# rustformers/llm

Hardware: NVIDIA B200
Metric: LLaMA-7B Q4_0 tokens/sec (decode@1, n_past=512) (higher is better)
Workload: dtype u8/s8 block dots -> f32 (Q4_0 weights x Q8_0 activations)

## Files before the change

llm_b200/csrc/decode_ops.cu:

```cuda
#include <cooperative_groups.h>
#include <stdlib.h>

#include <array>
#include <map>
#include <vector>

#include "decode.h"
#include "stream_core.cuh"
#include "tp.cuh"

namespace b200 {

using namespace stream;

__constant__ TpCtx c_tp;

namespace {

__device__ __forceinline__ unsigned long long gtime() { unsigned long long t; asm volatile("mov.u64 %0, %%globaltimer;" : "=l"(t)); return t; }
__device__ __forceinline__ void prof_begin(unsigned long long *p) { if (p && threadIdx.x == 0) { const unsigned long long t = gtime(); atomicMin(p, t); atomicMax(p + 3 * B200_PROF_SLOTS, t); } }
__device__ __forceinline__ void prof_ready(unsigned long long *p) { if (p && threadIdx.x == 0) { const unsigned long long t = gtime(); atomicMin(p + 2 * B200_PROF_SLOTS, t); atomicMax(p + 4 * B200_PROF_SLOTS, t); } }
__device__ __forceinline__ void prof_end(unsigned long long *p) { if (p && threadIdx.x == 0) atomicMax(p + B200_PROF_SLOTS, gtime()); }

__device__ __forceinline__ void pdl_trigger() { asm volatile("griddepcontrol.launch_dependents;" ::: "memory"); }
__device__ __forceinline__ void pdl_wait() { asm volatile("griddepcontrol.wait;" ::: "memory"); }

int pdl_mask() {
    static int mask = -1;
    if (mask < 0) { const char *e = getenv("B200_PDL"); mask = e ? atoi(e) : 3; }
    return mask;
}

template <int CLASS = 2, typename... KArgs, typename... Args>
void launch_k(void (*kern)(KArgs...), dim3 grid, dim3 block, size_t smem, cudaStream_t st, Args &&...args) {
    cudaLaunchConfig_t cfg{};
    cfg.gridDim = grid; cfg.blockDim = block; cfg.dynamicSmemBytes = smem; cfg.stream = st;
    cudaLaunchAttribute at[1];
    at[0].id = cudaLaunchAttributeProgrammaticStreamSerialization;
    at[0].val.programmaticStreamSerializationAllowed = 1;
    cfg.attrs = at; cfg.numAttrs = (pdl_mask() & CLASS) ? 1 : 0;
    B200_CHECK(cudaLaunchKernelEx(&cfg, kern, KArgs(args)...));
}

__device__ __forceinline__ float lutf(const uint16_t *t, float x) { return f16_bits_to_f32(__ldg(t + f32_to_f16_bits(x))); }
__device__ __forceinline__ float f16dot_tree(float s) {
    s = __fadd_rn(s, __shfl_down_sync(0xffffffffu, s, 16));
    s = __fadd_rn(s, __shfl_down_sync(0xffffffffu, s, 8));
    s = __fadd_rn(s, __shfl_down_sync(0xffffffffu, s, 4));
    s = __fadd_rn(s, __shfl_down_sync(0xffffffffu, s, 1));
    s = __fadd_rn(s, __shfl_down_sync(0xffffffffu, s, 2));
    return s;
}

template <bool TP>
__device__ __forceinline__ void norm_pack_body(const float *__restrict__ x, const float *__restrict__ gain, int4 *__restrict__ pack,
                                               int e, float eps, int q81, int off, int scale16, unsigned long long *prof, const TpSync &S) {
    const TpCtx &T = c_tp;
    __shared__ double shd[8];
    const int tid = threadIdx.x, lane = tid & 31, warp = tid >> 5;
    pdl_trigger();
    if (!(TP && (T.relax & 1))) pdl_wait();
    constexpr bool tp = TP;
    const unsigned tag = tp ? tp_tag(T, S.in_v) : 0u;

    prof_begin(prof);
    const int mine = blockIdx.x * 256 + tid, nv = e / 4;
    const bool active = mine < nv;
    const float4 gv = active ? __ldg((const float4 *)gain + mine) : make_float4(0.f, 0.f, 0.f, 0.f);
    float4 xv = make_float4(0.f, 0.f, 0.f, 0.f);
    double s = 0.0;
    constexpr int U = 4;
    if (tp && (T.relax & 1)) {
        if (warp == 0) tp_wait_sample(T, S.in_buf, (int64_t)e, tag, lane);
        __syncthreads();
    }
    for (int i0 = tid; i0 < nv; i0 += 256 * U) {
        float4 v[U];
        if (!tp) {
#pragma unroll
            for (int k = 0; k < U; k++) { const int i = i0 + 256 * k; v[k] = i < nv ? __ldcg((const float4 *)x + i) : make_float4(0.f, 0.f, 0.f, 0.f); }
        } else {
            uint4 ra[U], rb[U];
#pragma unroll
// ... 269 lines not shown
#pragma unroll
    for (int cc = 0; cc < 8; cc++) acc[cc] = 0.f;
    for (int k0 = 0; k0 < np; k0 += KC) {
        __syncthreads();
#pragma unroll
        for (int u = 0; u < KC / 32; u++) ((int4 *)vt)[tid + u * 128] = pre[u];
        __syncthreads();
        if (k0 + KC < np) fetch(k0 + KC);
        const int kend = np - k0 < KC ? np - k0 : KC;
#pragma unroll
        for (int cc = 0; cc < 8; cc++) {
            const __half *vrow = vt + (warp * 8 + cc) * KC;
            for (int k = lane; k < kend; k += 32) acc[cc] = __fmaf_rn(__half2float(vrow[k]), __half2float(p16[k0 + k]), acc[cc]);
        }
    }
    __syncthreads();
#pragma unroll
    for (int cc = 0; cc < 8; cc++) {
        const float a = f16dot_tree(acc[cc]);
        if (lane == 0) {
            const __half *vrow = vleft + (warp * 8 + cc) * 32;
            double sumf = (double)a;
            for (int k = np; k < n_kv; k++) sumf += (double)__fmul_rn(__half2float(vrow[k - np]), __half2float(p16[k]));
            stash[warp * 8 + cc] = (float)sumf;
        }
    }
    __syncthreads();
    if (warp == 0) pack_quad(((const float4 *)stash)[lane & 7], xpack_out + (int64_t)((h * hd + c0) / QK) * 4, lane, lane < 8, q81, off, scale16);
    prof_end(prof);
}

__device__ __forceinline__ float quad_tree(float (&acc)[8]) {
#pragma unroll
    for (int e = 0; e < 8; e++) acc[e] = __fadd_rn(acc[e], __shfl_xor_sync(0xffffffffu, acc[e], 2));
#pragma unroll
    for (int e = 0; e < 8; e++) acc[e] = __fadd_rn(acc[e], __shfl_xor_sync(0xffffffffu, acc[e], 1));
    const float r0 = __fadd_rn(acc[0], acc[4]), r1 = __fadd_rn(acc[1], acc[5]), r2 = __fadd_rn(acc[2], acc[6]), r3 = __fadd_rn(acc[3], acc[7]);
    return __fadd_rn(__fadd_rn(r0, r1), __fadd_rn(r2, r3));
}
__device__ __forceinline__ void fma8(float (&acc)[8], const int4 &a, const int4 &b) {
    const __half2 *ah = (const __half2 *)&a, *bh = (const __half2 *)&b;
#pragma unroll
    for (int e = 0; e < 4; e++) {
        const float2 af = __half22float2(ah[e]), bf = __half22float2(bh[e]);
        acc[2 * e] = __fmaf_rn(af.x, bf.x, acc[2 * e]); acc[2 * e + 1] = __fmaf_rn(af.y, bf.y, acc[2 * e + 1]);
    }
}

constexpr int ATH = 256;
template <bool TP>
__global__ void __launch_bounds__(ATH) attn_fused_kernel(const float *__restrict__ q, const __half *__restrict__ Kl, const __half *__restrict__ Vl,
                                                         int4 *__restrict__ xpack_out, const int *__restrict__ n_past, const uint16_t *__restrict__ lut_exp,
                                                         float kq_scale, int hd, int n_head, int n_head_kv, int gqa, int n_ctx, int nlay, int q81, int off, int scale16,
                                                         unsigned long long *prof, const TpSync S, int head0) {
    const TpCtx &T = c_tp;
    namespace cg = cooperative_groups;
    cg::cluster_group cluster = cg::this_cluster();
    extern __shared__ __align__(16) uint8_t sm[];
    __shared__ double shd[ATH / 32];
    __shared__ float shf[ATH / 32], stash[32];
    prof_begin(prof);
    const int per_head = hd / 32, h = blockIdx.x / per_head, part = blockIdx.x - h * per_head, c0 = part * 32;
    const int hk = h / (n_head / n_head_kv);
    const int tid = threadIdx.x, lane = tid & 31, warp = tid >> 5, u = tid & 3;
    const int vstride = nlay + 32;
    float *sc = (float *)sm;
    __half *p16 = (__half *)(sm + (size_t)nlay * 4);
    __half *q16 = p16 + nlay;
    __half *vs = (__half *)(sm + (((size_t)nlay * 6 + (size_t)hd * 2 + 127) & ~(size_t)127));
    pdl_trigger();
    pdl_wait();
    float qv = 0.f;
    if (tid < hd) qv = __ldcg(q + h * hd + tid);
    const int n_kv = __ldcg(n_past) + 1;
    const int np = n_kv & ~31;

    {
        const int cpr = (n_kv + 7) / 8;
        for (int i = tid; i < 32 * cpr; i += ATH) {
            const int rr = i / cpr, cc = i - rr * cpr;
            cp16(smem_u32(vs + rr * vstride + cc * 8), Vl + (int64_t)(hk * hd + c0 + rr) * n_ctx + cc * 8);
        }
    }
    if (tid < hd) q16[tid] = __float2half_rn(qv);
    __syncthreads();
    asm volatile("barrier.cluster.arrive.relaxed.aligned;\n\tbarrier.cluster.wait.aligned;" ::: "memory");

    {
        const int per = (n_kv + per_head - 1) / per_head, j0 = part * per, j1 = n_kv < j0 + per ? n_kv : j0 + per;
        const int nvec = hd / 32;
        constexpr int PU = 4;
        for (int jb = j0; jb < j1; jb += PU * (ATH / 4)) {
            int4 kv[PU][4];
#pragma unroll
            for (int pu = 0; pu < PU; pu++) {
                const int j = jb + pu * (ATH / 4) + (tid >> 2);
                const __half *krow = Kl + (int64_t)(j < j1 ? j : j0) * gqa + hk * hd + 8 * u;
#pragma unroll
                for (int i = 0; i < 4; i++) if (i < nvec) kv[pu][i] = j < j1 ? __ldcg((const int4 *)(krow + 32 * i)) : make_int4(0, 0, 0, 0);
            }
#pragma unroll
            for (int pu = 0; pu < PU; pu++) {
                const int j = jb + pu * (ATH / 4) + (tid >> 2);
                float acc[8];
#pragma unroll
                for (int e = 0; e < 8; e++) acc[e] = 0.f;
#pragma unroll
                for (int i = 0; i < 4; i++) if (i < nvec) fma8(acc, kv[pu][i], *(const int4 *)(q16 + 32 * i + 8 * u));
                const float s = quad_tree(acc);
                if (j < j1 && u < per_head) cluster.map_shared_rank(sc, u)[j] = __fmul_rn(s, kq_scale);
            }
        }
    }
    cluster.sync();

    float mx = -INFINITY;
    for (int j = tid; j < n_kv; j += ATH) mx = fmaxf(mx, sc[j]);
    mx = warp_max(mx);
    if (lane == 0) shf[warp] = mx;
    __syncthreads();
    mx = shf[0];
#pragma unroll
    for (int i = 1; i < ATH / 32; i++) mx = fmaxf(mx, shf[i]);
    double s = 0.0;
    constexpr int SB = 4;
    for (int jb = 0; jb < n_kv; jb += SB * ATH) {
        uint16_t ev16[SB];
#pragma unroll
        for (int k = 0; k < SB; k++) { const int j = jb + tid + k * ATH; ev16[k] = j < n_kv ? __ldg(lut_exp + f32_to_f16_bits(__fsub_rn(sc[j], mx))) : (uint16_t)0; }
#pragma unroll
        for (int k = 0; k < SB; k++) { const int j = jb + tid + k * ATH; if (j < n_kv) { const float ev = f16_bits_to_f32(ev16[k]); sc[j] = ev; s += (double)ev; } }
    }
    s = warp_sum(s);
    if (lane == 0) shd[warp] = s;
    __syncthreads();
    const float inv = (float)(1.0 / (((shd[0] + shd[1]) + (shd[2] + shd[3])) + ((shd[4] + shd[5]) + (shd[6] + shd[7]))));
    for (int j = tid; j < n_kv; j += ATH) p16[j] = __float2half_rn(__fmul_rn(sc[j], inv));
    asm volatile("cp.async.wait_all;" ::: "memory");
    __syncthreads();

    if (tid < 128) {
        const int col = tid >> 2;
        const __half *vrow = vs + col * vstride;
        float acc[8];
#pragma unroll
        for (int e = 0; e < 8; e++) acc[e] = 0.f;
#pragma unroll 4
        for (int k = 0; k < np; k += 32) fma8(acc, *(const int4 *)(vrow + k + 8 * u), *(const int4 *)(p16 + k + 8 * u));
        const float a = quad_tree(acc);
        if (u == 0) {
            double sumf = (double)a;
            for (int k = np; k < n_kv; k++) sumf += (double)__fmul_rn(__half2float(vrow[k]), __half2float(p16[k]));
            stash[col] = (float)sumf;
        }
    }
    __syncthreads();
    if (warp == 0) {
        int4 rec;
        const int64_t blk = (int64_t)(((head0 + h) * hd + c0) / QK);
        if (pack_quad_rec(((const float4 *)stash)[lane & 7], lane, lane < 8, q81, off, scale16, rec)) {
            if (TP) tp_put_rec(T, TPB_XD, blk * 4 + (lane & 7), rec, tp_tag(T, S.out_v)); else xpack_out[blk * 4 + (lane & 7)] = rec;
        }
    }
    prof_end(prof);
}

template <int TYPE, int EPI, bool TP = false>
void launch_mmv(const QWeight &w, MmvArgs A, cudaStream_t st) {
    constexpr int ROWS = SR, CB = SCB;
    using T = St<TYPE>;
    static int smem_set = 0, sms = 0, depth_cap = -1;
    static std::map<int, std::array<int, SST_MAX + 1>> occ_by_nb;
    if (!sms) { int dev; B200_CHECK(cudaGetDevice(&dev)); B200_CHECK(cudaDeviceGetAttribute(&sms, cudaDevAttrMultiProcessorCount, dev)); }
    if (depth_cap < 0) { const char *e = getenv("B200_RING_DEPTH"); depth_cap = e ? atoi(e) : SST_MAX; if (depth_cap < 2) depth_cap = 2; if (depth_cap > SST_MAX) depth_cap = SST_MAX; }
    auto smem_of = [&](int nst) { return 256 + T::ring_bytes(nst) + (int)w.nb * 64 + 256; };
    if (smem_of(SST_MAX) > smem_set) {
        const int want = smem_of(SST_MAX) < 227 * 1024 ? smem_of(SST_MAX) : 227 * 1024;
        B200_CHECK(cudaFuncSetAttribute(mmv_fused_kernel<TYPE, EPI, TP>, cudaFuncAttributeMaxDynamicSharedMemorySize, want));
        smem_set = smem_of(SST_MAX);
    }
    auto it = occ_by_nb.find((int)w.nb);
    if (it == occ_by_nb.end()) {
        std::array<int, SST_MAX + 1> o{};
        for (int nst = 2; nst <= SST_MAX; nst++)
            if (smem_of(nst) <= 227 * 1024) B200_CHECK(cudaOccupancyMaxActiveBlocksPerMultiprocessor(&o[nst], mmv_fused_kernel<TYPE, EPI, TP>, STHREADS, smem_of(nst)));
        it = occ_by_nb.emplace((int)w.nb, o).first;
    }
    const std::array<int, SST_MAX + 1> &occ = it->second;
    constexpr int G = EPI == EPI_SILU ? 2 : 1;
    const int64_t groups = ((w.N + ROWS - 1) / ROWS + G - 1) / G;
// ... 38 lines not shown
    if (threadIdx.x == 0) *T.epoch = *(volatile unsigned *)T.epoch + 1;
}

template <int TYPE, bool TP>
void decode_ops_t(const DecodeParams &P, const std::vector<DecodeLayer> &layers, int n_kv_bucket, int4 *xpack_a, cudaStream_t st, int *launches) {
    const int q81 = has_min(TYPE) ? 1 : 0, off = TYPE == T_Q5_0 ? 16 : 0, s16 = TYPE == T_Q4_0 ? 1 : 0;
    const int e = P.e, f = P.f;
    const TpCtx &T = P.tp;
    constexpr bool tp = TP;
    B200_ASSERT(tp == (T.world > 1));
    const int e_loc = tp ? P.e_loc : e;
    auto ts = [&](int in_buf, unsigned in_v, int add_buf, unsigned add_v, int out_buf, unsigned out_v) {
        TpSync S;
        if (tp) { S.in_buf = in_buf; S.in_v = in_v; S.add_buf = add_buf; S.add_v = add_v; S.out_buf = out_buf; S.out_v = out_v; }
        return S;
    };
    int n = 0;
    auto pr = [&]() -> unsigned long long * { return P.prof && n < B200_PROF_SLOTS ? P.prof + n : nullptr; };
    auto launch_norm = [&](const float *x, const float *gain, const TpSync &S) {
        const dim3 grid((e / QK + 31) / 32), block(256);
        if constexpr (TP) launch_k(norm_pack_tp_kernel, grid, block, 0, st, x, gain, xpack_a, e, P.eps, q81, off, s16, pr(), S);
        else { (void)S; launch_k(norm_pack_kernel, grid, block, 0, st, x, gain, xpack_a, e, P.eps, q81, off, s16, pr()); }
        n++;
    };
    get_rows_q(P.wte, P.token, P.x, 1, st); n++;
    if (tp) { launch_k(tp_spread_kernel, dim3((e + 255) / 256), dim3(256), 0, st, (const float *)P.x, e); n++; }
    static const bool fused_env = !(getenv("B200_ATTN_FUSED") && getenv("B200_ATTN_FUSED")[0] == '0');
    const int nlay = (n_kv_bucket + 63) / 64 * 64;
    const size_t fa_smem = (((size_t)nlay * 6 + (size_t)P.hd * 2 + 127) & ~(size_t)127) + (size_t)32 * (nlay + 32) * 2;
    const bool fused_attn = (fused_env || tp) && P.hd % 32 == 0 && P.hd <= 128 && P.n_ctx % 8 == 0 && fa_smem <= 227 * 1024;
    B200_ASSERT(fused_attn || !tp);
    if (fused_attn) attn_fused_reserve(fa_smem);
    const size_t sv_smem = (size_t)P.n_ctx * 6 + 32 * KC * 2 + 32 * 32 * 2;
    static size_t sv_set = 48 * 1024;
    if (sv_smem > sv_set) { B200_CHECK(cudaFuncSetAttribute(attn_sv_kernel, cudaFuncAttributeMaxDynamicSharedMemorySize, (int)sv_smem)); sv_set = sv_smem; }
    for (int il = 0; il < P.n_layer; il++) {
        const DecodeLayer &L = layers[il];
        const unsigned v = (unsigned)il + 1;
        launch_norm(P.x, L.attn_norm, ts(TPB_X, (unsigned)il, -1, 0, -1, 0));
        MmvArgs A{}; A.xpack = xpack_a; A.q = P.q; A.K = L.K; A.V = L.V; A.rope_cs = P.rope_cs; A.rope_half = P.rope_half; A.hd = P.hd; A.e = e_loc; A.gqa = P.gqa;
        A.n_ctx = P.n_ctx; A.n_past = P.n_past;
        A.prof = pr(); launch_mmv<TYPE, EPI_QKV, TP>(L.wqkv, A, st); n++;
        if (fused_attn) {
            cudaLaunchConfig_t cfg{};
            cfg.gridDim = dim3(P.n_head * (P.hd / 32)); cfg.blockDim = dim3(ATH); cfg.dynamicSmemBytes = fa_smem; cfg.stream = st;
            cudaLaunchAttribute at[2];
            at[0].id = cudaLaunchAttributeClusterDimension;
            at[0].val.clusterDim.x = P.hd / 32; at[0].val.clusterDim.y = 1; at[0].val.clusterDim.z = 1;
            at[1].id = cudaLaunchAttributeProgrammaticStreamSerialization;
            at[1].val.programmaticStreamSerializationAllowed = 1;
            cfg.attrs = at; cfg.numAttrs = (pdl_mask() & 2) ? 2 : 1;
            B200_CHECK(cudaLaunchKernelEx(&cfg, attn_fused_kernel<TP>, (const float *)P.q, (const __half *)L.K, (const __half *)L.V, P.xpack_d, (const int *)P.n_past,
                                          (const uint16_t *)P.lut_exp, P.kq_scale, P.hd, P.n_head, P.n_head_kv, P.gqa, P.n_ctx, nlay, q81, off, s16, pr(),
                                          ts(-1, 0, -1, 0, TPB_XD, v), tp ? P.head0 : 0));
            n++;
        } else {
            launch_k(P.hd == 128 ? attn_kq_kernel<128> : attn_kq_kernel<64>, dim3((n_kv_bucket + 63) / 64, P.n_head), dim3(128), 0, st,
                     P.q, L.K, P.kq, P.n_past, P.gqa, P.n_head, P.n_head_kv, P.n_ctx, pr());
            n++;
            launch_k(attn_sv_kernel, dim3(P.n_head * (P.hd / 32)), dim3(128), sv_smem, st, P.kq, L.V, P.xpack_d, P.n_past, P.lut_exp, P.kq_scale, P.hd, P.n_head,
                     P.n_head_kv, P.n_ctx, q81, off, s16, pr()); n++;
        }
        MmvArgs Bo{}; Bo.xpack = P.xpack_d; Bo.dst = P.ff; Bo.addend = P.x;
        Bo.ts = ts(TPB_XD, v, TPB_X, (unsigned)il, TPB_FF, v); Bo.row0 = tp ? P.row0_e : 0;
        Bo.prof = pr(); launch_mmv<TYPE, EPI_RES, TP>(L.wo, Bo, st); n++;
        launch_norm(P.ff, L.ffn_norm, ts(TPB_FF, v, -1, 0, -1, 0));
        MmvArgs C{}; C.xpack = xpack_a; C.xpack_out = P.xpack_f; C.lut_silu = P.lut_silu; C.q81 = q81; C.off = off; C.scale16 = s16;
        C.ts = ts(-1, 0, -1, 0, TPB_XF, v); C.row0 = tp ? P.row0_w13 : 0;
        C.prof = pr(); launch_mmv<TYPE, EPI_SILU, TP>(L.w13, C, st); n++;
        MmvArgs D{}; D.xpack = P.xpack_f; D.dst = P.x; D.addend = P.ff;
        D.ts = ts(TPB_XF, v, TPB_FF, v, TPB_X, v); D.row0 = tp ? P.row0_e : 0;
        D.prof = pr(); launch_mmv<TYPE, EPI_RES, TP>(L.w2, D, st); n++;
    }
    launch_norm(P.x, P.norm, ts(TPB_X, (unsigned)P.n_layer, -1, 0, -1, 0));
    MmvArgs Z{}; Z.xpack = xpack_a; Z.dst = P.logits; Z.addend = nullptr; Z.n_past_inc = P.n_past;
    Z.ts = ts(-1, 0, -1, 0, TPB_LOGITS, 0); Z.row0 = tp ? P.row0_v : 0;
    Z.prof = pr(); launch_mmv<TYPE, EPI_LOGITS, TP>(P.output, Z, st); n++;
    if (tp) {
        launch_k(tp_collect_kernel, dim3((P.n_vocab_full + 255) / 256), dim3(256), 0, st, P.logits, P.n_vocab_full); n++;
        launch_k(tp_bump_kernel, dim3(1), dim3(32), 0, st); n++;
    }
    B200_CHECK(cudaGetLastError());
    (void)f;
    if (launches) *launches = n;
}

__global__ void __launch_bounds__(256) ln_pack_kernel(const float *__restrict__ x, const float *__restrict__ gain, const float *__restrict__ bias, int4 *__restrict__ pack,
                                                      int e, int q81, int off, int scale16) {
    __shared__ double shd[8];
    const int tid = threadIdx.x, lane = tid & 31, warp = tid >> 5;
    pdl_trigger();
    pdl_wait();
    constexpr int MAXV = 8;
    const int nv = e / 4, mine = blockIdx.x * 256 + tid;
    float4 v[MAXV];
#pragma unroll
    for (int k = 0; k < MAXV; k++) { const int i = tid + k * 256; v[k] = i < nv ? __ldcg((const float4 *)x + i) : make_float4(0.f, 0.f, 0.f, 0.f); }
    const bool active = mine < nv;
    const float4 gv = active ? __ldg((const float4 *)gain + mine) : make_float4(0.f, 0.f, 0.f, 0.f);
    const float4 bv = active ? __ldg((const float4 *)bias + mine) : make_float4(0.f, 0.f, 0.f, 0.f);
    auto total = [&](double s) {
        s = warp_sum(s);
        __syncthreads();
        if (lane == 0) shd[warp] = s;
        __syncthreads();
        return ((shd[0] + shd[1]) + (shd[2] + shd[3])) + ((shd[4] + shd[5]) + (shd[6] + shd[7]));
    };
// ... 32 lines not shown
    if (n_rot > 0) {
        const int hb = n_rot / 2, ib = c / n_rot, r = c - ib * n_rot;
        if (ib < hd / n_rot) {
            const bool lo = r < hb;
            const int partner = lo ? c + hb : c - hb;
            const float2 cs = __ldg(rope_cs + (int64_t)p * rope_half + ib * hb + (lo ? r : r - hb));
            const float qp = __ldcg(base + partner), kp = __ldcg(base + k_off + partner);
            qo = lo ? __fmaf_rn(qo, cs.x, -__fmul_rn(qp, cs.y)) : __fmaf_rn(qp, cs.y, __fmul_rn(qo, cs.x));
            ko = lo ? __fmaf_rn(ko, cs.x, -__fmul_rn(kp, cs.y)) : __fmaf_rn(kp, cs.y, __fmul_rn(ko, cs.x));
        }
    }
    q[i] = qo;
    Kl[(int64_t)p * e + i] = __float2half_rn(ko);
    Vl[(int64_t)i * n_ctx + p] = __float2half_rn(__ldcg(base + v_off + c));
}

__global__ void __launch_bounds__(256) gpt2_add_pos_kernel(float *__restrict__ x, const float *__restrict__ wpe, const int *__restrict__ n_past, int e) {
    pdl_wait();
    const int i = blockIdx.x * 256 + threadIdx.x;
    if (i < e) x[i] = __fadd_rn(x[i], __ldg(wpe + (int64_t)__ldcg(n_past) * e + i));
}

template <int TYPE>
void neox_ops_t(const NeoxParams &P, const std::vector<NeoxLayer> &layers, int n_kv_bucket, cudaStream_t st, int *launches) {
    const int q81 = has_min(TYPE) ? 1 : 0, off = TYPE == T_Q5_0 ? 16 : 0, s16 = TYPE == T_Q4_0 ? 1 : 0;
    const int e = P.e;
    int n = 0;
    get_rows_q(P.wte, P.token, P.x, 1, st); n++;
    if (P.wpe) { launch_k(gpt2_add_pos_kernel, dim3((e + 255) / 256), dim3(256), 0, st, P.x, P.wpe, (const int *)P.n_past, e); n++; }
    const int nlay = (n_kv_bucket + 63) / 64 * 64;
    const size_t fa_smem = (((size_t)nlay * 6 + (size_t)P.hd * 2 + 127) & ~(size_t)127) + (size_t)32 * (nlay + 32) * 2;
    B200_ASSERT(P.hd % 32 == 0 && P.hd <= 128 && P.n_ctx % 8 == 0 && fa_smem <= 227 * 1024 && e <= 8192);
    attn_fused_reserve(fa_smem);
    const dim3 ln_grid((e / 4 + 255) / 256);
    const TpSync S{};
    for (int il = 0; il < P.n_layer; il++) {
        const NeoxLayer &L = layers[il];
        launch_k(ln_pack_kernel, ln_grid, dim3(256), 0, st, (const float *)P.x, L.ln1_g, L.ln1_b, P.xpack_a, e, q81, off, s16); n++;
        MmvArgs A{}; A.xpack = P.xpack_a; A.dst = P.qkv; A.bias = L.bqkv;
        launch_mmv<TYPE, EPI_BIAS>(L.wqkv, A, st); n++;
        launch_k(neox_rope_store_kernel, dim3((e + 255) / 256), dim3(256), 0, st, (const float *)P.qkv, P.q, L.K, L.V, (const int *)P.n_past, P.rope_cs, P.rope_half,
                 P.gpt2 ? 0 : P.n_rot, P.hd, e, P.n_ctx, P.gpt2 ? P.hd : 3 * P.hd, P.gpt2 ? e : P.hd, P.gpt2 ? 2 * e : 2 * P.hd); n++;
        {
            cudaLaunchConfig_t cfg{};
            cfg.gridDim = dim3(P.n_head * (P.hd / 32)); cfg.blockDim = dim3(ATH); cfg.dynamicSmemBytes = fa_smem; cfg.stream = st;
            cudaLaunchAttribute at[2];
            at[0].id = cudaLaunchAttributeClusterDimension;
            at[0].val.clusterDim.x = P.hd / 32; at[0].val.clusterDim.y = 1; at[0].val.clusterDim.z = 1;
            at[1].id = cudaLaunchAttributeProgrammaticStreamSerialization;
            at[1].val.programmaticStreamSerializationAllowed = 1;
            cfg.attrs = at; cfg.numAttrs = (pdl_mask() & 2) ? 2 : 1;
            B200_CHECK(cudaLaunchKernelEx(&cfg, attn_fused_kernel<false>, (const float *)P.q, (const __half *)L.K, (const __half *)L.V, P.xpack_d, (const int *)P.n_past,
                                          (const uint16_t *)P.lut_exp, P.kq_scale, P.hd, P.n_head, P.n_head, e, P.n_ctx, nlay, q81, off, s16,
                                          (unsigned long long *)nullptr, S, 0));
            n++;
        }
        MmvArgs Bo{}; Bo.xpack = P.xpack_d; Bo.dst = P.attn_out; Bo.bias = L.bdense; Bo.add1 = P.parallel_residual ? nullptr : P.x;
        launch_mmv<TYPE, EPI_BIAS>(L.wdense, Bo, st); n++;
        launch_k(ln_pack_kernel, ln_grid, dim3(256), 0, st, (const float *)(P.parallel_residual ? P.x : P.attn_out), L.ln2_g, L.ln2_b, P.xpack_a, e, q81, off, s16); n++;
        MmvArgs C{}; C.xpack = P.xpack_a; C.xpack_out = P.xpack_f; C.bias = L.bfc; C.lut_gelu = P.lut_gelu; C.q81 = q81; C.off = off; C.scale16 = s16;
        launch_mmv<TYPE, EPI_GELU>(L.wfc, C, st); n++;
        MmvArgs D{}; D.xpack = P.xpack_f; D.dst = P.x; D.bias = L.bproj; D.add1 = P.attn_out; D.add2 = P.parallel_residual ? P.x : nullptr;
        launch_mmv<TYPE, EPI_BIAS>(L.wproj, D, st); n++;
    }
    launch_k(ln_pack_kernel, ln_grid, dim3(256), 0, st, (const float *)P.x, P.lnf_g, P.lnf_b, P.xpack_a, e, q81, off, s16); n++;
    MmvArgs Z{}; Z.xpack = P.xpack_a; Z.dst = P.logits; Z.n_past_inc = P.n_past;
    launch_mmv<TYPE, EPI_BIAS>(P.lm_head, Z, st); n++;
    B200_CHECK(cudaGetLastError());
    if (launches) *launches = n;
}

}

void neox_decode_enqueue(const NeoxParams &P, const std::vector<NeoxLayer> &layers, int wtype, int n_kv_bucket, cudaStream_t st, int *launches) {
    switch (wtype) {
        case T_Q4_0: neox_ops_t<T_Q4_0>(P, layers, n_kv_bucket, st, launches); break;
        case T_Q4_1: neox_ops_t<T_Q4_1>(P, layers, n_kv_bucket, st, launches); break;
        case T_Q5_0: neox_ops_t<T_Q5_0>(P, layers, n_kv_bucket, st, launches); break;
        case T_Q5_1: neox_ops_t<T_Q5_1>(P, layers, n_kv_bucket, st, launches); break;
        case T_Q8_0: neox_ops_t<T_Q8_0>(P, layers, n_kv_bucket, st, launches); break;
        default: B200_ASSERT(!"neox_decode_enqueue: unsupported weight type");
    }
}

void decode_set_tp(const TpCtx &T, cudaStream_t st) {
    B200_CHECK(cudaStreamSynchronize(st));
    B200_CHECK(cudaMemcpyToSymbol(c_tp, &T, sizeof(TpCtx)));
    B200_CHECK(cudaDeviceSynchronize());
}

void decode_ops_enqueue(const DecodeParams &P, const std::vector<DecodeLayer> &layers, int wtype, int n_kv_bucket, int4 *xpack_a, cudaStream_t st, int *launches) {
    const bool tp = P.tp.world > 1;
    switch (wtype) {
        case T_Q4_0: if (tp) decode_ops_t<T_Q4_0, true>(P, layers, n_kv_bucket, xpack_a, st, launches); else decode_ops_t<T_Q4_0, false>(P, layers, n_kv_bucket, xpack_a, st, launches); break;
        case T_Q4_1: if (tp) decode_ops_t<T_Q4_1, true>(P, layers, n_kv_bucket, xpack_a, st, launches); else decode_ops_t<T_Q4_1, false>(P, layers, n_kv_bucket, xpack_a, st, launches); break;
        case T_Q5_0: if (tp) decode_ops_t<T_Q5_0, true>(P, layers, n_kv_bucket, xpack_a, st, launches); else decode_ops_t<T_Q5_0, false>(P, layers, n_kv_bucket, xpack_a, st, launches); break;
        case T_Q5_1: if (tp) decode_ops_t<T_Q5_1, true>(P, layers, n_kv_bucket, xpack_a, st, launches); else decode_ops_t<T_Q5_1, false>(P, layers, n_kv_bucket, xpack_a, st, launches); break;
        case T_Q8_0: if (tp) decode_ops_t<T_Q8_0, true>(P, layers, n_kv_bucket, xpack_a, st, launches); else decode_ops_t<T_Q8_0, false>(P, layers, n_kv_bucket, xpack_a, st, launches); break;
        default: B200_ASSERT(!"decode_ops_enqueue: unsupported weight type");
    }
}

}
```

llm_b200/csrc/session.cu:

```cuda
#include <string.h>

#include <string>
#include <vector>

#include "../../include/llm_b200.h"
#include "decode.h"
#include "kernels.cuh"
#include "runtime.h"

namespace b200 {
void synth_qweight(const QWeight &w, uint64_t seed, cudaStream_t st);
void synth_gain(float *g, int64_t n, uint64_t seed, cudaStream_t st);
}
using namespace b200;

namespace {

QWeight row_view(const QWeight &w, int64_t row0, int64_t nrows) {
    QWeight v = w;
    v.N = nrows;
    v.qs = w.qs + (size_t)row0 * w.nb * qs_bytes(w.type);
    if (w.qh) v.qh = w.qh + (size_t)row0 * w.nb;
    v.dm = (const uint8_t *)w.dm + (size_t)row0 * w.nb * (has_min(w.type) ? 4 : 2);
    v.base = nullptr;
// ... 437 lines not shown
        B200_CHECK(cudaStreamSynchronize(R.stream));
    } else {
        if (nbytes != (size_t)s.n * 4) return B200_ERR_TENSOR_SHAPE;
        B200_CHECK(cudaStreamSynchronize(R.stream));
        B200_CHECK(cudaMemcpy(host_out, s.f, nbytes, cudaMemcpyDeviceToHost));
    }
    return B200_OK;
}

int b200_model_synthesize(b200_model *m, uint64_t seed) {
    if (!m || m->tp_world > 1) return B200_ERR_BAD_ARG;
    cudaStream_t st = rt().stream;
    uint64_t id = 0;
    auto q = [&](const QWeight &w) { synth_qweight(w, seed + 0x1000003ull * (++id), st); };
    auto g = [&](float *p, int64_t n) { synth_gain(p, n, seed + 0x1000003ull * (++id), st); };
    q(m->wte); g(m->norm, m->hp.n_embd); q(m->output);
    for (auto &L : m->layers) { g(L.attention_norm, m->hp.n_embd); g(L.ffn_norm, m->hp.n_embd); q(L.wqkv); q(L.wo); q(L.w13); q(L.w2); }
    B200_CHECK(cudaStreamSynchronize(st));
    m->loaded.assign(m->n_slots(), 1);
    m->n_loaded = m->n_slots();
    return B200_OK;
}

int b200_model_is_loaded(b200_model *m) { return m && m->n_loaded == m->n_slots(); }

void b200_model_free(b200_model *m) {
    if (!m) return;
    B200_CHECK(cudaStreamSynchronize(rt().stream));
    if (m->slab) B200_CHECK(cudaFree(m->slab));
    delete m;
}

static b200_session *start_session_tp(b200_session *s) {
    b200_model *m = s->m;
    const b200_llama_hparams &hp = m->hp;
    const int G = m->tp_world, r = m->tp_rank;
    const size_t e = hp.n_embd, f = hp.n_ff, n_ctx = hp.context_size, gqa = m->gqa_loc, V = hp.n_vocab;
    s->cfg.n_batch = s->cfg.n_batch < 1 ? 1 : s->cfg.n_batch;
    const size_t kv_elems = (size_t)hp.n_layer * n_ctx * gqa;
    B200_CHECK(cudaMalloc(&s->memory_k, kv_elems * 2));
    B200_CHECK(cudaMalloc(&s->memory_v, kv_elems * 2));
    B200_CHECK(cudaMemset(s->memory_k, 0, kv_elems * 2));
    B200_CHECK(cudaMemset(s->memory_v, 0, kv_elems * 2));
    B200_CHECK(cudaMalloc(&s->d_tokens, (size_t)s->cfg.n_batch * 4));
    B200_CHECK(cudaMallocHost(&s->h_tokens, (size_t)s->cfg.n_batch * 4));
    B200_CHECK(cudaMallocHost(&s->h_logits, (size_t)s->cfg.n_batch * V * 4));
    B200_CHECK(cudaMallocHost(&s->h_topk, 2048 * 4));
    B200_CHECK(cudaMalloc(&s->topk, 2048 * 4));
    B200_CHECK(cudaEventCreateWithFlags(&s->tokens_uploaded, cudaEventDisableTiming));
    B200_CHECK(cudaMalloc(&s->qbuf, (size_t)m->e_loc * 4));
    B200_CHECK(cudaMalloc(&s->xpack_a, (e / QK) * 64));
    B200_CHECK(cudaMalloc(&s->d_n_past, sizeof(int)));
    B200_CHECK(cudaMallocHost(&s->h_n_past, sizeof(int)));
    B200_CHECK(cudaMalloc(&s->d_prof, B200_PROF_SLOTS * 8 * sizeof(unsigned long long)));
    B200_CHECK(cudaMemset(s->d_prof, 0, B200_PROF_SLOTS * 8 * sizeof(unsigned long long)));
    TpCtx &T = s->dp.tp;
    T = TpCtx();
    T.world = G; T.rank = r; T.vmul = (unsigned)hp.n_layer + 1;
    { const char *e = getenv("B200_TP_RELAX"); T.relax = e ? atoi(e) : 0; }
    size_t off = 0;
    auto piece = [&](size_t units) { const size_t o = off; off += (units * 8 + 255) & ~(size_t)255; return (uint32_t)o; };
    T.off[TPB_X] = piece(e); T.off[TPB_FF] = piece(e); T.off[TPB_XD] = piece((e / QK) * 16); T.off[TPB_XF] = piece((f / QK) * 16); T.off[TPB_LOGITS] = piece(V);
    s->tp_slab_bytes = off;
    B200_CHECK(cudaMalloc(&s->tp_slab, off));
    B200_CHECK(cudaMemset(s->tp_slab, 0, off));
    B200_CHECK(cudaMalloc(&s->tp_state, 2 * sizeof(unsigned)));
    B200_CHECK(cudaMemset(s->tp_state, 0, 2 * sizeof(unsigned)));
    T.epoch = s->tp_state;
    for (int p = 0; p < TP_MAX; p++) T.peer[p] = nullptr;
    T.peer[r] = s->tp_slab;
    B200_CHECK(cudaMalloc(&s->x, e * 4));
    B200_CHECK(cudaMalloc(&s->logits, V * 4));
    s->ff = nullptr; s->xpack_d = nullptr; s->xpack_f = nullptr;
    const RopeTable &rt_ = rope_table(hp.n_rot, 0, hp.rope_freq_base, hp.rope_freq_scale, m->hd, (int)n_ctx);
    {
        std::vector<DecodeLayer> hl(hp.n_layer);
        for (int il = 0; il < hp.n_layer; il++) {
            const Layer &L = m->layers[il];
            hl[il] = DecodeLayer{L.wqkv, L.wo, L.w13, L.w2, L.attention_norm, L.ffn_norm,
                                 s->memory_k + (size_t)il * n_ctx * gqa, s->memory_v + (size_t)il * n_ctx * gqa};
        }
        s->h_layers = hl;
    }
    DecodeParams &P = s->dp;
    P.layers = nullptr; P.n_layer = hp.n_layer; P.wte = m->wte; P.output = m->output; P.norm = m->norm;
    P.e = (int)e; P.f = m->f_loc; P.hd = m->hd; P.gqa = m->gqa_loc; P.n_head = hp.n_head / G; P.n_head_kv = hp.n_head_kv / G; P.n_ctx = (int)n_ctx; P.n_vocab = m->v_loc;
    P.kq_scale = 1.0f / sqrtf((float)hp.n_embd / (float)hp.n_head); P.eps = 5e-6f;
    P.rope_cs = rt_.cs; P.rope_half = rt_.half;
    P.lut_silu = luts().silu; P.lut_exp = luts().exp;
    P.token = s->d_tokens; P.n_past = s->d_n_past;
    P.x = s->x; P.q = s->qbuf; P.kq = nullptr; P.attn = nullptr; P.ff = s->ff; P.h13 = nullptr; P.logits = s->logits;
    P.xpack_d = s->xpack_d; P.xpack_f = s->xpack_f; P.bar = nullptr; P.scratch_bytes = 0;
    P.e_loc = m->e_loc; P.head0 = r * (hp.n_head / G); P.n_vocab_full = hp.n_vocab;
    P.row0_e = (int64_t)r * m->e_loc; P.row0_w13 = (int64_t)r * 2 * m->f_loc; P.row0_v = (int64_t)r * m->v_loc;
    P.prof = nullptr;
    QWeight probe; probe.nb = (int64_t)e / QK;
    QWeight probe2; probe2.nb = (int64_t)f / QK;
    s->mega_ok = hp.n_rot == m->hd && (m->hd == 64 || m->hd == 128) && mmv_exact_stream_supported(probe) && mmv_exact_stream_supported(probe2) &&
                 m->gqa_loc % 32 == 0 && m->e_loc % 32 == 0 && hp.context_size % 8 == 0;
    B200_CHECK(cudaDeviceSynchronize());
    if (!s->mega_ok) { fprintf(stderr, "llm_b200: tensor-parallel session: geometry not supported by the fused decode schedule\n"); b200_session_free(s); return nullptr; }
    return s;
}

b200_session *b200_model_start_session(b200_model *m, const b200_session_config *cfg) {
    if (!m || !cfg || cfg->n_batch < 1) return nullptr;
    if (m->n_loaded != m->n_slots()) { fprintf(stderr, "llm_b200: start_session: %d of %d tensors loaded\n", m->n_loaded, m->n_slots()); return nullptr; }
    b200_session *s = new b200_session();
// ... 7 lines not shown
    B200_CHECK(cudaMemset(s->memory_k, 0, kv_elems * 2));
    B200_CHECK(cudaMemset(s->memory_v, 0, kv_elems * 2));
    const size_t kmax = e > f ? e : f;
    B200_CHECK(cudaMalloc(&s->d_tokens, B * 4));
    B200_CHECK(cudaMalloc(&s->x, B * e * 4));
    B200_CHECK(cudaMalloc(&s->cur, B * e * 4));
    B200_CHECK(cudaMalloc(&s->ff, B * e * 4));
    B200_CHECK(cudaMalloc(&s->qkv, B * (e + 2 * gqa) * 4));
    B200_CHECK(cudaMalloc(&s->kq, (size_t)hp.n_head * B * n_ctx * 4));
    B200_CHECK(cudaMalloc(&s->h13, B * 2 * f * 4));
    B200_CHECK(cudaMalloc(&s->hmul, B * f * 4));
    B200_CHECK(cudaMalloc(&s->logits, B * (size_t)hp.n_vocab * 4));
    B200_CHECK(cudaMalloc(&s->xq, B * kmax));
    B200_CHECK(cudaMalloc(&s->topk, 2048 * 4));
    B200_CHECK(cudaMalloc(&s->xds, B * (kmax / QK) * sizeof(float2)));
    B200_CHECK(cudaMalloc(&s->xpack, (kmax / QK) * 64));
    B200_CHECK(cudaMalloc(&s->xh, xh_bytes(kmax, B)));
    B200_CHECK(cudaMallocHost(&s->h_tokens, B * 4));
    B200_CHECK(cudaMallocHost(&s->h_logits, B * (size_t)hp.n_vocab * 4));
    B200_CHECK(cudaMallocHost(&s->h_topk, 2048 * 4));
    B200_CHECK(cudaEventCreateWithFlags(&s->tokens_uploaded, cudaEventDisableTiming));
    const RopeTable &rt_ = rope_table(hp.n_rot, 0, hp.rope_freq_base, hp.rope_freq_scale, m->hd, (int)n_ctx);
    B200_CHECK(cudaMalloc(&s->qbuf, e * 4));
    B200_CHECK(cudaMalloc(&s->attn, e * 4));
    B200_CHECK(cudaMalloc(&s->d_bar, 2 * sizeof(unsigned int)));
    B200_CHECK(cudaMemset(s->d_bar, 0, 2 * sizeof(unsigned int)));
    B200_CHECK(cudaMalloc(&s->d_n_past, sizeof(int)));
    B200_CHECK(cudaMallocHost(&s->h_n_past, sizeof(int)));
    {
        std::vector<DecodeLayer> hl(hp.n_layer);
        for (int il = 0; il < hp.n_layer; il++) {
            const Layer &L = m->layers[il];
            hl[il] = DecodeLayer{L.wqkv, L.wo, L.w13, L.w2, L.attention_norm, L.ffn_norm,
                                 s->memory_k + (size_t)il * n_ctx * gqa, s->memory_v + (size_t)il * n_ctx * gqa};
        }
        s->h_layers = hl;
        B200_CHECK(cudaMalloc(&s->d_layers, hl.size() * sizeof(DecodeLayer)));
        B200_CHECK(cudaMemcpy(s->d_layers, hl.data(), hl.size() * sizeof(DecodeLayer), cudaMemcpyHostToDevice));
    }
    DecodeParams &P = s->dp;
    P.layers = s->d_layers; P.n_layer = hp.n_layer; P.wte = m->wte; P.output = m->output; P.norm = m->norm;
    P.e = (int)e; P.f = (int)f; P.hd = m->hd; P.gqa = m->gqa; P.n_head = hp.n_head; P.n_head_kv = hp.n_head_kv; P.n_ctx = (int)n_ctx; P.n_vocab = hp.n_vocab;
    P.kq_scale = 1.0f / sqrtf((float)hp.n_embd / (float)hp.n_head); P.eps = 5e-6f;
    P.rope_cs = rt_.cs; P.rope_half = rt_.half;
    P.lut_silu = luts().silu; P.lut_exp = luts().exp;
    P.token = s->d_tokens; P.n_past = s->d_n_past;
    P.x = s->x; P.q = s->qbuf; P.kq = s->kq; P.attn = s->attn; P.ff = s->ff; P.h13 = s->h13; P.logits = s->logits;
    P.bar = s->d_bar;
    B200_CHECK(cudaMalloc(&s->xpack_d, (e / QK) * 64));
    B200_CHECK(cudaMalloc(&s->xpack_f, (f / QK) * 64));
    P.xpack_d = s->xpack_d; P.xpack_f = s->xpack_f;
    B200_CHECK(cudaMalloc(&s->xpack_a, (e / QK) * 64));
    P.scratch_bytes = decode_scratch_bytes((int)e, (int)f, m->hd, (int)n_ctx);
    B200_CHECK(cudaMalloc(&s->d_prof, B200_PROF_SLOTS * 8 * sizeof(unsigned long long)));
    B200_CHECK(cudaMemset(s->d_prof, 0, B200_PROF_SLOTS * 8 * sizeof(unsigned long long)));
    P.prof = getenv("B200_DECODE_PROF") ? s->d_prof : nullptr;
    s->mega_ok = hp.n_rot == m->hd && (m->hd == 64 || m->hd == 128) && decode_supported(P, hp.wtype);
    B200_CHECK(cudaDeviceSynchronize());
    return s;
}

int32_t b200_session_n_past(const b200_session *s) { return s ? s->n_past : -1; }
int b200_session_set_n_past(b200_session *s, int32_t n_past) {
    if (!s || n_past < 0 || n_past > s->n_past) return B200_ERR_BAD_ARG;
    s->n_past = n_past;
    return B200_OK;
}
int32_t b200_session_last_launches(const b200_session *s) { return s ? s->last_launches : 0; }

int b200_session_evaluate_device(b200_session *s, const int32_t *d_tokens, int32_t n) {
    if (!s || n < 1 || n > s->cfg.n_batch) return B200_ERR_BAD_ARG;
    if (s->n_past + n > s->m->hp.context_size) return B200_ERR_CONTEXT_FULL;
    if (d_tokens && d_tokens != s->d_tokens)
        B200_CHECK(cudaMemcpyAsync(s->d_tokens, d_tokens, (size_t)n * 4, cudaMemcpyDeviceToDevice, rt().stream));
    forward(s, n);
    return B200_OK;
}
const float *b200_session_device_logits(b200_session *s) { return s ? s->logits : nullptr; }

int b200_session_evaluate(b200_session *s, const int32_t *tokens, int32_t n, float *logits_out, int32_t all_logits) {
    if (!s || !tokens || n < 1 || n > s->cfg.n_batch) return B200_ERR_BAD_ARG;
    if (s->n_past + n > s->m->hp.context_size) return B200_ERR_CONTEXT_FULL;
    if (s->m->tp_world > 1 && n > 1) {
        const size_t V = s->m->hp.n_vocab;
        for (int i = 0; i < n; i++) {
            float *out = !logits_out ? nullptr : all_logits ? logits_out + (size_t)i * V : (i == n - 1 ? logits_out : nullptr);
            const int rc = b200_session_evaluate(s, tokens + i, 1, out, 0);
            if (rc != B200_OK) return rc;
        }
        return B200_OK;
    }
    for (int i = 0; i < n; i++) if (tokens[i] < 0 || tokens[i] >= s->m->hp.n_vocab) return B200_ERR_BAD_ARG;
    cudaStream_t st = rt().stream;
    B200_CHECK(cudaEventSynchronize(s->tokens_uploaded));
    memcpy(s->h_tokens, tokens, (size_t)n * 4);
    B200_CHECK(cudaMemcpyAsync(s->d_tokens, s->h_tokens, (size_t)n * 4, cudaMemcpyHostToDevice, st));
    B200_CHECK(cudaEventRecord(s->tokens_uploaded, st));
    forward(s, n, all_logits != 0);
    const size_t V = s->m->hp.n_vocab;
    if (logits_out) {
        const size_t rows = all_logits ? n : 1;
        const float *src = all_logits ? s->logits : s->logits + (size_t)(n - 1) * V;
        B200_CHECK(cudaMemcpyAsync(s->h_logits, src, rows * V * 4, cudaMemcpyDeviceToHost, st));
        B200_CHECK(cudaStreamSynchronize(st));
        memcpy(logits_out, s->h_logits, rows * V * 4);
    }
    return B200_OK;
}
// ... 8 lines not shown
    B200_CHECK(cudaMemcpyAsync(s->h_topk, d_ids, (size_t)k * 4, cudaMemcpyDeviceToHost, st));
    B200_CHECK(cudaMemcpyAsync(s->h_topk + 1024, d_vals, (size_t)k * 4, cudaMemcpyDeviceToHost, st));
    B200_CHECK(cudaStreamSynchronize(st));
    memcpy(ids_out, s->h_topk, (size_t)k * 4);
    memcpy(logits_out, s->h_topk + 1024, (size_t)k * 4);
    return B200_OK;
}

int b200_session_feed_prompt(b200_session *s, const int32_t *tokens, int32_t n, float *last_logits_out) {
    if (!s || !tokens || n < 0) return B200_ERR_BAD_ARG;
    if (s->n_past + n > s->m->hp.context_size) return B200_ERR_CONTEXT_FULL;
    for (int i = 0; i < n; i += s->cfg.n_batch) {
        const int c = (n - i) < s->cfg.n_batch ? (n - i) : s->cfg.n_batch;
        const bool last = i + c >= n;
        const int rc = b200_session_evaluate(s, tokens + i, c, last ? last_logits_out : nullptr, 0);
        if (rc != B200_OK) return rc;
    }
    return B200_OK;
}

int b200_session_read_kv(b200_session *s, int32_t which, void *host_out, size_t nbytes) {
    if (!s || !host_out) return B200_ERR_BAD_ARG;
    const size_t kv_bytes = (size_t)s->m->hp.n_layer * s->m->hp.context_size * (s->m->tp_world > 1 ? s->m->gqa_loc : s->m->gqa) * 2;
    if (nbytes != kv_bytes) return B200_ERR_TENSOR_SHAPE;
    B200_CHECK(cudaStreamSynchronize(rt().stream));
    B200_CHECK(cudaMemcpy(host_out, which ? s->memory_v : s->memory_k, kv_bytes, cudaMemcpyDeviceToHost));
    return B200_OK;
}

int b200_session_set_tap(b200_session *s, int32_t layer, int32_t stage) {
    if (!s || s->m->tp_world > 1) return B200_ERR_BAD_ARG;
    s->tap_layer = layer; s->tap_stage = stage; s->tap_count = 0;
    return B200_OK;
}
int64_t b200_session_read_tap(b200_session *s, float *host_out, int64_t max_count) {
    if (!s || !host_out) return B200_ERR_BAD_ARG;
    B200_CHECK(cudaStreamSynchronize(rt().stream));
    const size_t c = s->tap_count < (size_t)max_count ? s->tap_count : (size_t)max_count;
    if (c) B200_CHECK(cudaMemcpy(host_out, s->tap, c * 4, cudaMemcpyDeviceToHost));
    return (int64_t)c;
}

int b200_session_decode_profile(b200_session *s, unsigned long long *out128) {
    if (!s || !out128) return B200_ERR_BAD_ARG;
    B200_CHECK(cudaStreamSynchronize(rt().stream));
    B200_CHECK(cudaMemcpy(out128, s->d_prof, 128 * sizeof(unsigned long long), cudaMemcpyDeviceToHost));
    return B200_OK;
}

int b200_session_decode_timeline(b200_session *s, unsigned long long *out, int n, int reset) {
    if (!s || n < 0 || n > B200_PROF_SLOTS) return B200_ERR_BAD_ARG;
    B200_CHECK(cudaStreamSynchronize(rt().stream));
    if (out && n) {
        for (int k = 0; k < 8; k++)
            B200_CHECK(cudaMemcpy(out + (size_t)k * n, s->d_prof + (size_t)k * B200_PROF_SLOTS, (size_t)n * sizeof(unsigned long long), cudaMemcpyDeviceToHost));
    }
    if (reset) {
        for (int k = 0; k < 8; k++)
            B200_CHECK(cudaMemset(s->d_prof + (size_t)k * B200_PROF_SLOTS, (k == 0 || k == 2 || k == 5) ? 0xFF : 0, B200_PROF_SLOTS * sizeof(unsigned long long)));
        B200_CHECK(cudaDeviceSynchronize());
    }
    return B200_OK;
}

int b200_session_sync(b200_session *s) { (void)s; B200_CHECK(cudaStreamSynchronize(rt().stream)); return B200_OK; }

int b200_session_tp_handle(b200_session *s, void *handle_out64) {
    if (!s || !s->tp_slab || !handle_out64) return B200_ERR_BAD_ARG;
    static_assert(sizeof(cudaIpcMemHandle_t) == 64, "handle size");
    cudaIpcMemHandle_t h;
    B200_CHECK(cudaIpcGetMemHandle(&h, s->tp_slab));
    memcpy(handle_out64, &h, 64);
    return B200_OK;
}
int b200_session_tp_connect(b200_session *s, const void *handles_by_rank) {
    if (!s || !s->tp_slab || !handles_by_rank) return B200_ERR_BAD_ARG;
    TpCtx &T = s->dp.tp;
    for (int p = 0; p < T.world; p++) {
        if (p == T.rank) continue;
        cudaIpcMemHandle_t h;
        memcpy(&h, (const char *)handles_by_rank + (size_t)p * 64, 64);
        void *ptr = nullptr;
        const cudaError_t err = cudaIpcOpenMemHandle(&ptr, h, cudaIpcMemLazyEnablePeerAccess);
        if (err != cudaSuccess) { fprintf(stderr, "llm_b200: cudaIpcOpenMemHandle(rank %d): %s\n", p, cudaGetErrorString(err)); return B200_ERR_IO; }
        s->tp_peer_map[p] = ptr;
        T.peer[p] = (char *)ptr;
    }
    s->tp_connected = true;
    decode_set_tp(T, rt().stream);
    return B200_OK;
}
int b200_session_tp_set_nowait(b200_session *s, int32_t nowait) {
    if (!s || !s->tp_slab) return B200_ERR_BAD_ARG;
    B200_CHECK(cudaStreamSynchronize(rt().stream));
    s->dp.tp.nowait = nowait < 0 ? 0 : nowait > 2 ? 2 : nowait;
    decode_set_tp(s->dp.tp, rt().stream);
    for (auto &g : s->graphs) cudaGraphExecDestroy(g.second);
    s->graphs.clear();
    return B200_OK;
}
int32_t b200_session_tp_timeouts(b200_session *s) {
    if (!s || !s->tp_state) return -1;
    unsigned v[2] = {0, 0};
    B200_CHECK(cudaStreamSynchronize(rt().stream));
    B200_CHECK(cudaMemcpy(v, s->tp_state, sizeof(v), cudaMemcpyDeviceToHost));
    return (int32_t)v[1];
}

void b200_session_free(b200_session *s) {
    if (!s) return;
    B200_CHECK(cudaStreamSynchronize(rt().stream));
// ... 170 lines not shown
```

Measured before the change: 575.8.

## Prefetch past KV cache rows in attention before the PDL grid-dependency wait

The fused attention kernel now issues loads for the already-written K rows (positions before the current token) into registers and starts cp.async copies of the old V columns before calling griddepcontrol.wait. After the wait it loads only the newly written K row and the remaining V chunk. The goal is to overlap KV-cache memory traffic with the tail of the preceding kernel under programmatic dependent launch. It relies on earlier KV rows not being modified by the upstream kernel. It also adds profiling timestamps and a ninth profiling slot, and can be disabled with an environment variable.

Measured after the change: 593.4, median of 6. 1.03x the previous value.

```diff
diff --git a/llm_b200/csrc/decode_ops.cu b/llm_b200/csrc/decode_ops.cu
--- a/llm_b200/csrc/decode_ops.cu
+++ b/llm_b200/csrc/decode_ops.cu
@@ -21,6 +21,9 @@
 __device__ __forceinline__ void prof_begin(unsigned long long *p) { if (p && threadIdx.x == 0) { const unsigned long long t = gtime(); atomicMin(p, t); atomicMax(p + 3 * B200_PROF_SLOTS, t); } }
 __device__ __forceinline__ void prof_ready(unsigned long long *p) { if (p && threadIdx.x == 0) { const unsigned long long t = gtime(); atomicMin(p + 2 * B200_PROF_SLOTS, t); atomicMax(p + 4 * B200_PROF_SLOTS, t); } }
 __device__ __forceinline__ void prof_end(unsigned long long *p) { if (p && threadIdx.x == 0) atomicMax(p + B200_PROF_SLOTS, gtime()); }
+__device__ __forceinline__ void prof_stamp(unsigned long long *p, int kmin, int kmax) {
+    if (p && threadIdx.x == 0) { const unsigned long long t = gtime(); if (kmin >= 0) atomicMin(p + kmin * B200_PROF_SLOTS, t); atomicMax(p + kmax * B200_PROF_SLOTS, t); }
+}
 
 __device__ __forceinline__ void pdl_trigger() { asm volatile("griddepcontrol.launch_dependents;" ::: "memory"); }
 __device__ __forceinline__ void pdl_wait() { asm volatile("griddepcontrol.wait;" ::: "memory"); }
@@ -29,6 +32,11 @@
     static int mask = -1;
     if (mask < 0) { const char *e = getenv("B200_PDL"); mask = e ? atoi(e) : 3; }
     return mask;
+}
+int attn_prefetch() {
+    static int on = -1;
+    if (on < 0) { const char *e = getenv("B200_ATTN_PREFETCH"); on = e ? (atoi(e) != 0) : 1; }
+    return on;
 }
 
 template <int CLASS = 2, typename... KArgs, typename... Args>
@@ -404,7 +412,7 @@
 __global__ void __launch_bounds__(ATH) attn_fused_kernel(const float *__restrict__ q, const __half *__restrict__ Kl, const __half *__restrict__ Vl,
                                                          int4 *__restrict__ xpack_out, const int *__restrict__ n_past, const uint16_t *__restrict__ lut_exp,
                                                          float kq_scale, int hd, int n_head, int n_head_kv, int gqa, int n_ctx, int nlay, int q81, int off, int scale16,
-                                                         unsigned long long *prof, const TpSync S, int head0) {
+                                                         unsigned long long *prof, const TpSync S, int head0, int prefetch) {
     const TpCtx &T = c_tp;
     namespace cg = cooperative_groups;
     cg::cluster_group cluster = cg::this_cluster();
@@ -421,50 +429,71 @@
     __half *q16 = p16 + nlay;
     __half *vs = (__half *)(sm + (((size_t)nlay * 6 + (size_t)hd * 2 + 127) & ~(size_t)127));
     pdl_trigger();
-    pdl_wait();
+    if (!prefetch) { pdl_wait(); prof_ready(prof); }
+    const int n_kv = __ldcg(n_past) + 1, p = n_kv - 1;
+    const int np = n_kv & ~31;
+
+    const int cpr = (n_kv + 7) / 8;
+    auto copy_v = [&](int c_lo, int c_hi) {
+        const int nc = c_hi - c_lo;
+        for (int i = tid; i < 32 * nc; i += ATH) {
+            const int rr = i / nc, cc = c_lo + i - rr * nc;
+            cp16(smem_u32(vs + rr * vstride + cc * 8), Vl + (int64_t)(hk * hd + c0 + rr) * n_ctx + cc * 8);
+        }
+    };
+    const int vpre = prefetch ? p / 8 : 0;
+
+    const int per = (n_kv + per_head - 1) / per_head, j0 = part * per, j1 = n_kv < j0 + per ? n_kv : j0 + per;
+    const int nvec = hd / 32;
+    constexpr int PU = 4;
+    int4 kv[PU][4];
+    auto load_k = [&](int jb, int jend) {
+#pragma unroll
+        for (int pu = 0; pu < PU; pu++) {
+            const int j = jb + pu * (ATH / 4) + (tid >> 2);
+            const __half *krow = Kl + (int64_t)(j < jend ? j : j0) * gqa + hk * hd + 8 * u;
+#pragma unroll
+            for (int i = 0; i < 4; i++) if (i < nvec) kv[pu][i] = j < jend ? __ldcg((const int4 *)(krow + 32 * i)) : make_int4(0, 0, 0, 0);
+        }
+    };
+    load_k(j0, prefetch ? (p < j1 ? p : j1) : 0);
+    copy_v(0, vpre);
+    asm volatile("barrier.cluster.arrive.relaxed.aligned;\n\tbarrier.cluster.wait.aligned;" ::: "memory");
+    if (prefetch) { pdl_wait(); prof_ready(prof); }
+
     float qv = 0.f;
     if (tid < hd) qv = __ldcg(q + h * hd + tid);
-    const int n_kv = __ldcg(n_past) + 1;
-    const int np = n_kv & ~31;
-
-    {
-        const int cpr = (n_kv + 7) / 8;
-        for (int i = tid; i < 32 * cpr; i += ATH) {
-            const int rr = i / cpr, cc = i - rr * cpr;
-            cp16(smem_u32(vs + rr * vstride + cc * 8), Vl + (int64_t)(hk * hd + c0 + rr) * n_ctx + cc * 8);
-        }
-    }
+    if (!prefetch) load_k(j0, j1);
+    else {
+#pragma unroll
+        for (int pu = 0; pu < PU; pu++)
+            if (j0 + pu * (ATH / 4) + (tid >> 2) == p) {
+                const __half *krow = Kl + (int64_t)p * gqa + hk * hd + 8 * u;
+#pragma unroll
+                for (int i = 0; i < 4; i++) if (i < nvec) kv[pu][i] = __ldcg((const int4 *)(krow + 32 * i));
+            }
+    }
+    copy_v(vpre, cpr);
     if (tid < hd) q16[tid] = __float2half_rn(qv);
     __syncthreads();
-    asm volatile("barrier.cluster.arrive.relaxed.aligned;\n\tbarrier.cluster.wait.aligned;" ::: "memory");
-
-    {
-        const int per = (n_kv + per_head - 1) / per_head, j0 = part * per, j1 = n_kv < j0 + per ? n_kv : j0 + per;
-        const int nvec = hd / 32;
-        constexpr int PU = 4;
-        for (int jb = j0; jb < j1; jb += PU * (ATH / 4)) {
-            int4 kv[PU][4];
-#pragma unroll
-            for (int pu = 0; pu < PU; pu++) {
-                const int j = jb + pu * (ATH / 4) + (tid >> 2);
-                const __half *krow = Kl + (int64_t)(j < j1 ? j : j0) * gqa + hk * hd + 8 * u;
-#pragma unroll
-                for (int i = 0; i < 4; i++) if (i < nvec) kv[pu][i] = j < j1 ? __ldcg((const int4 *)(krow + 32 * i)) : make_int4(0, 0, 0, 0);
-            }
-#pragma unroll
-            for (int pu = 0; pu < PU; pu++) {
-                const int j = jb + pu * (ATH / 4) + (tid >> 2);
-                float acc[8];
-#pragma unroll
-                for (int e = 0; e < 8; e++) acc[e] = 0.f;
-#pragma unroll
-                for (int i = 0; i < 4; i++) if (i < nvec) fma8(acc, kv[pu][i], *(const int4 *)(q16 + 32 * i + 8 * u));
-                const float s = quad_tree(acc);
-                if (j < j1 && u < per_head) cluster.map_shared_rank(sc, u)[j] = __fmul_rn(s, kq_scale);
-            }
-        }
-    }
+
+    for (int jb = j0; jb < j1; jb += PU * (ATH / 4)) {
+        if (jb != j0) load_k(jb, j1);
+#pragma unroll
+        for (int pu = 0; pu < PU; pu++) {
+            const int j = jb + pu * (ATH / 4) + (tid >> 2);
+            float acc[8];
+#pragma unroll
+            for (int e = 0; e < 8; e++) acc[e] = 0.f;
+#pragma unroll
+            for (int i = 0; i < 4; i++) if (i < nvec) fma8(acc, kv[pu][i], *(const int4 *)(q16 + 32 * i + 8 * u));
+            const float s = quad_tree(acc);
+            if (j < j1 && u < per_head) cluster.map_shared_rank(sc, u)[j] = __fmul_rn(s, kq_scale);
+        }
+    }
+    prof_stamp(prof, 5, 6);
     cluster.sync();
+    prof_stamp(prof, -1, 7);
 
     float mx = -INFINITY;
     for (int j = tid; j < n_kv; j += ATH) mx = fmaxf(mx, sc[j]);
@@ -488,6 +517,7 @@
     __syncthreads();
     const float inv = (float)(1.0 / (((shd[0] + shd[1]) + (shd[2] + shd[3])) + ((shd[4] + shd[5]) + (shd[6] + shd[7]))));
     for (int j = tid; j < n_kv; j += ATH) p16[j] = __float2half_rn(__fmul_rn(sc[j], inv));
+    prof_stamp(prof, -1, 8);
     asm volatile("cp.async.wait_all;" ::: "memory");
     __syncthreads();
 
@@ -632,7 +662,7 @@
             cfg.attrs = at; cfg.numAttrs = (pdl_mask() & 2) ? 2 : 1;
             B200_CHECK(cudaLaunchKernelEx(&cfg, attn_fused_kernel<TP>, (const float *)P.q, (const __half *)L.K, (const __half *)L.V, P.xpack_d, (const int *)P.n_past,
                                           (const uint16_t *)P.lut_exp, P.kq_scale, P.hd, P.n_head, P.n_head_kv, P.gqa, P.n_ctx, nlay, q81, off, s16, pr(),
-                                          ts(-1, 0, -1, 0, TPB_XD, v), tp ? P.head0 : 0));
+                                          ts(-1, 0, -1, 0, TPB_XD, v), tp ? P.head0 : 0, attn_prefetch()));
             n++;
         } else {
             launch_k(P.hd == 128 ? attn_kq_kernel<128> : attn_kq_kernel<64>, dim3((n_kv_bucket + 63) / 64, P.n_head), dim3(128), 0, st,
@@ -771,7 +801,7 @@
             cfg.attrs = at; cfg.numAttrs = (pdl_mask() & 2) ? 2 : 1;
             B200_CHECK(cudaLaunchKernelEx(&cfg, attn_fused_kernel<false>, (const float *)P.q, (const __half *)L.K, (const __half *)L.V, P.xpack_d, (const int *)P.n_past,
                                           (const uint16_t *)P.lut_exp, P.kq_scale, P.hd, P.n_head, P.n_head, e, P.n_ctx, nlay, q81, off, s16,
-                                          (unsigned long long *)nullptr, S, 0));
+                                          (unsigned long long *)nullptr, S, 0, attn_prefetch()));
             n++;
         }
         MmvArgs Bo{}; Bo.xpack = P.xpack_d; Bo.dst = P.attn_out; Bo.bias = L.bdense; Bo.add1 = P.parallel_residual ? nullptr : P.x;
diff --git a/llm_b200/csrc/session.cu b/llm_b200/csrc/session.cu
--- a/llm_b200/csrc/session.cu
+++ b/llm_b200/csrc/session.cu
@@ -513,8 +513,8 @@
     B200_CHECK(cudaMalloc(&s->xpack_a, (e / QK) * 64));
     B200_CHECK(cudaMalloc(&s->d_n_past, sizeof(int)));
     B200_CHECK(cudaMallocHost(&s->h_n_past, sizeof(int)));
-    B200_CHECK(cudaMalloc(&s->d_prof, B200_PROF_SLOTS * 8 * sizeof(unsigned long long)));
-    B200_CHECK(cudaMemset(s->d_prof, 0, B200_PROF_SLOTS * 8 * sizeof(unsigned long long)));
+    B200_CHECK(cudaMalloc(&s->d_prof, B200_PROF_SLOTS * 9 * sizeof(unsigned long long)));
+    B200_CHECK(cudaMemset(s->d_prof, 0, B200_PROF_SLOTS * 9 * sizeof(unsigned long long)));
     TpCtx &T = s->dp.tp;
     T = TpCtx();
     T.world = G; T.rank = r; T.vmul = (unsigned)hp.n_layer + 1;
@@ -628,8 +628,8 @@
     P.xpack_d = s->xpack_d; P.xpack_f = s->xpack_f;
     B200_CHECK(cudaMalloc(&s->xpack_a, (e / QK) * 64));
     P.scratch_bytes = decode_scratch_bytes((int)e, (int)f, m->hd, (int)n_ctx);
-    B200_CHECK(cudaMalloc(&s->d_prof, B200_PROF_SLOTS * 8 * sizeof(unsigned long long)));
-    B200_CHECK(cudaMemset(s->d_prof, 0, B200_PROF_SLOTS * 8 * sizeof(unsigned long long)));
+    B200_CHECK(cudaMalloc(&s->d_prof, B200_PROF_SLOTS * 9 * sizeof(unsigned long long)));
+    B200_CHECK(cudaMemset(s->d_prof, 0, B200_PROF_SLOTS * 9 * sizeof(unsigned long long)));
     P.prof = getenv("B200_DECODE_PROF") ? s->d_prof : nullptr;
     s->mega_ok = hp.n_rot == m->hd && (m->hd == 64 || m->hd == 128) && decode_supported(P, hp.wtype);
     B200_CHECK(cudaDeviceSynchronize());
@@ -744,11 +744,11 @@
     if (!s || n < 0 || n > B200_PROF_SLOTS) return B200_ERR_BAD_ARG;
     B200_CHECK(cudaStreamSynchronize(rt().stream));
     if (out && n) {
-        for (int k = 0; k < 8; k++)
+        for (int k = 0; k < 9; k++)
             B200_CHECK(cudaMemcpy(out + (size_t)k * n, s->d_prof + (size_t)k * B200_PROF_SLOTS, (size_t)n * sizeof(unsigned long long), cudaMemcpyDeviceToHost));
     }
     if (reset) {
-        for (int k = 0; k < 8; k++)
+        for (int k = 0; k < 9; k++)
             B200_CHECK(cudaMemset(s->d_prof + (size_t)k * B200_PROF_SLOTS, (k == 0 || k == 2 || k == 5) ? 0xFF : 0, B200_PROF_SLOTS * sizeof(unsigned long long)));
         B200_CHECK(cudaDeviceSynchronize());
     }
```
